# ToniChopp/ECAMP

Hardware: AMD Instinct MI355X
Metric: pretrain image-report pairs/sec (ViT-B/16, 224^2, seq=128) (higher is better)
Workload: dtype bf16

## Files before the change

ecamp_amd/csrc/core.hip:

```cpp
#include "common.h"
#include "attention.h"
#include "options.h"
#include "../../include/ecamp_hip.h"
#include <atomic>
#include <stdarg.h>
#include <stdlib.h>

thread_local char g_ecamp_err[512] = {0};

int ecamp_set_error(int code, const char* fmt, ...) {
    va_list ap;
    va_start(ap, fmt);
    vsnprintf(g_ecamp_err, sizeof(g_ecamp_err), fmt, ap);
    va_end(ap);
    return code;
}

extern "C" const char* ecamp_last_error(void) { return g_ecamp_err; }
extern "C" int ecamp_abi_version(void) { return ECAMP_ABI_VERSION; }
extern "C" int ecamp_half_format(void) { return ECAMP_HALF_IS_F16; }

#define OPT_UNREAD (INT_MIN + 1)
struct OptRow {
    const char* name; const char* env; int def; int (*set)(int);
    std::atomic<int> value{OPT_ENV};
    std::atomic<int> env_value{OPT_UNREAD};
};
static OptRow g_opts[OPT_COUNT] = {
              {"q8_mode", "ECAMP_GEMM_Q8", -1, [](int v) { return v == 0 || v == 2 ? v : -1; }},
               {"q8_sch", "ECAMP_Q8_SCH", 7, [](int v) { return v >= 0 ? v : OPT_ENV; }},
             {"q16_mode", "ECAMP_Q16", 1, [](int v) { return v >= 0 && v <= 3 ? v : OPT_ENV; }},
                {nullptr, "ECAMP_F8_Q8", 1, nullptr},
         {nullptr, "ECAMP_Q8_MIN_ITEMS", OPT_AUTO, nullptr},
          {"q8_bwd_grid", "ECAMP_Q8_BWD_GRID", 0, [](int v) { return v > 0 ? v : OPT_ENV; }},
             {"p8_wgrad", nullptr, 1, [](int v) { return v ? 1 : 0; }},
     {"p8_wgrad_reserve_cus", nullptr, 0, [](int v) { return v < 0 ? 0 : v; }},
          {nullptr, "ECAMP_WGRAD_ITEMS", 0, nullptr},
           {nullptr, "ECAMP_WGRAD_PLAN", 1, nullptr},
      {nullptr, "ECAMP_WGRAD_GROUP_CUS", 0, nullptr},
        {nullptr, "ECAMP_GEMM_GRID_CAP", 0, nullptr},
            {"attn_head", "ECAMP_ATTN_HEAD", 1, [](int v) { return v < 0 ? OPT_ENV : v ? 1 : 0; }},
           {nullptr, "ECAMP_ATTN_WAVES", 0, nullptr},
               {nullptr, "ECAMP_LN_BWD", 0, nullptr},
            {nullptr, "ECAMP_CE_KERNEL", 1, nullptr},
            {nullptr, "ECAMP_SR_BLOCKS", 512, nullptr},
};
int ecamp_opt_default(EcampOpt id) { return g_opts[id].def; }
int ecamp_opt(EcampOpt id) {
    OptRow& o = g_opts[id];
    const int s = o.value.load(std::memory_order_relaxed);
    if (s != OPT_ENV) return s;
    int e = o.env_value.load(std::memory_order_relaxed);
    if (e == OPT_UNREAD) {
        const char* txt = o.env ? getenv(o.env) : nullptr;
        e = txt ? atoi(txt) : o.def;
        o.env_value.store(e, std::memory_order_relaxed);
    }
    return e;
}
bool ecamp_opt_set(const char* name, int value) {
    for (OptRow& o : g_opts)
        if (o.name && strcmp(name, o.name) == 0) {
            o.value.store(o.set(value), std::memory_order_relaxed);
            return true;
        }
    return false;
}
extern "C" int ecamp_set_option(const char* name, int32_t value) {
    ECAMP_CHECK_ARG(name != nullptr, "set_option: null name");
    if (strcmp(name, "attn_head") == 0) { attn_set_head_mode(value); return 0; }
    if (ecamp_opt_set(name, value)) return 0;
    return ecamp_set_error(-1, "set_option: unknown option '%s'", name);
}

__global__ void dev_spin_kernel(long long cycles) {
    const long long t0 = clock64();
    while (clock64() - t0 < cycles) {}
}
extern "C" int ecamp_dev_spin(int32_t blocks, int32_t threads, int64_t cycles, hipStream_t stream) {
    ECAMP_CHECK_ARG(blocks > 0 && threads > 0 && threads <= 1024 && cycles >= 0, "dev_spin: bad arguments");
    hipLaunchKernelGGL(dev_spin_kernel, dim3(blocks), dim3(threads), 0, stream, (long long)cycles);
    ECAMP_LAUNCH_CHECK();
    return 0;
}
```

ecamp_amd/csrc/norm.hip:

```cpp
#include "common.h"
#include <initializer_list>

template <typename T, int VEC> struct LnVec;
template <> struct LnVec<float, 4> {
    typedef float4 raw_t;
    static __device__ __forceinline__ void cvt(const float4& v, float (&o)[4]) { o[0] = v.x; o[1] = v.y; o[2] = v.z; o[3] = v.w; }
    static __device__ __forceinline__ float4 pack(const float (&o)[4]) { return make_float4(o[0], o[1], o[2], o[3]); }
};
template <> struct LnVec<float, 8> {
    struct raw_t { float4 a, b; };
    static __device__ __forceinline__ void cvt(const raw_t& v, float (&o)[8]) {
        o[0] = v.a.x; o[1] = v.a.y; o[2] = v.a.z; o[3] = v.a.w; o[4] = v.b.x; o[5] = v.b.y; o[6] = v.b.z; o[7] = v.b.w;
    }
};
template <> struct LnVec<bf16_t, 4> {
    typedef uint2 raw_t;
    static __device__ __forceinline__ void cvt(const uint2& v, float (&o)[4]) {
        o[0] = h16_lo(v.x); o[1] = h16_hi(v.x);
        o[2] = h16_lo(v.y); o[3] = h16_hi(v.y);
    }
    static __device__ __forceinline__ uint2 pack(const float (&o)[4]) { return make_uint2(pack_bf16x2(o[0], o[1]), pack_bf16x2(o[2], o[3])); }
};
template <> struct LnVec<bf16_t, 8> {
    typedef uint4 raw_t;
    static __device__ __forceinline__ void cvt(const uint4& v, float (&o)[8]) {
        o[0] = h16_lo(v.x); o[1] = h16_hi(v.x);
        o[2] = h16_lo(v.y); o[3] = h16_hi(v.y);
        o[4] = h16_lo(v.z); o[5] = h16_hi(v.z);
        o[6] = h16_lo(v.w); o[7] = h16_hi(v.w);
    }
    static __device__ __forceinline__ uint4 pack(const float (&o)[8]) {
        return make_uint4(pack_bf16x2(o[0], o[1]), pack_bf16x2(o[2], o[3]), pack_bf16x2(o[4], o[5]), pack_bf16x2(o[6], o[7]));
    }
};
template <int VEC>
__device__ __forceinline__ void ln_dropout(uint64_t seed, uint64_t offset, long row, int nv, int c, float p, float inv_keep, float (&m)[VEC]) {
    if constexpr (VEC == 8) {
        dropout_scale8(seed, offset, (uint64_t)(row * nv + c), p, inv_keep, m);
    } else {
        static_assert(VEC == 4, "ln_dropout: 4- or 8-wide chunks");
        dropout_scale4(seed, offset, (uint64_t)(row * nv + c), p, inv_keep, m);
    }
}

template <typename T> struct ln_z32 {};
template <typename T> struct LnRow { typedef T io; typedef T z; };
template <typename T> struct LnRow<ln_z32<T>> { typedef T io; typedef float z; };

template <typename T, int IT, int VEC>
__global__ __launch_bounds__(256) void ln_fwd_kernel(const T* __restrict__ x, const T* __restrict__ res, T* __restrict__ zout,
                                                     const float* __restrict__ gamma, const float* __restrict__ beta,
                                                     T* __restrict__ y, float* __restrict__ mean, float* __restrict__ rstd,
                                                     long rows, int cols, float eps, float drop_p, uint64_t seed,
                                                     uint64_t offset, unsigned char* __restrict__ q8, const float* __restrict__ q8_scale,
                                                     float* __restrict__ q8_amax) {
    typedef typename LnRow<T>::io TY;
    typedef typename LnRow<T>::z TX;
    typedef LnVec<TY, VEC> V;
    typedef LnVec<TX, VEC> VX;
    typedef typename V::raw_t raw_t;
    const int lane = threadIdx.x & 63;
    const long row = (long)blockIdx.x * 4 + (threadIdx.x >> 6);
    if (row >= rows) return;
    const float q8_inv = q8 ? 1.0f / fmaxf(q8_scale[0], 1e-30f) : 0.f;
    float q8_max = 0.f;
    const int nv = cols / VEC;
    const float inv_keep = drop_p > 0.f ? 1.0f / (1.0f - drop_p) : 1.0f;
    typename VX::raw_t rx[IT];
    raw_t rr[IT];
#pragma unroll
    for (int i = 0; i < IT; ++i) {
        const int c = lane + 64 * i;
        if (c < nv) {
            rx[i] = *reinterpret_cast<const typename VX::raw_t*>(reinterpret_cast<const TX*>(x) + row * cols + c * VEC);
            if (res) rr[i] = *reinterpret_cast<const raw_t*>(reinterpret_cast<const TY*>(res) + row * cols + c * VEC);
        }
    }
    float v[IT][VEC];
    float s = 0.f;
#pragma unroll
    for (int i = 0; i < IT; ++i) {
        const int c = lane + 64 * i;
        if (c < nv) {
            VX::cvt(rx[i], v[i]);
            if (drop_p > 0.f) {
                float m[VEC];
                ln_dropout<VEC>(seed, offset, row, nv, c, drop_p, inv_keep, m);
#pragma unroll
                for (int r = 0; r < VEC; ++r) v[i][r] *= m[r];
            }
            if (res) {
                float q[VEC];
                V::cvt(rr[i], q);
#pragma unroll
                for (int r = 0; r < VEC; ++r) v[i][r] += q[r];
            }
            if (zout) {
#pragma unroll
                for (int r = 0; r < VEC; ++r) v[i][r] = rnd<TY>(v[i][r]);
                *reinterpret_cast<raw_t*>(reinterpret_cast<TY*>(zout) + row * cols + c * VEC) = V::pack(v[i]);
            }
#pragma unroll
            for (int r = 0; r < VEC; r += 4) s += (v[i][r] + v[i][r + 1]) + (v[i][r + 2] + v[i][r + 3]);
        } else {
#pragma unroll
            for (int r = 0; r < VEC; ++r) v[i][r] = 0.f;
        }
    }
    const float mu = wave_sum(s) / (float)cols;
    float q = 0.f;
#pragma unroll
    for (int i = 0; i < IT; ++i) {
        const int c = lane + 64 * i;
        if (c < nv) {
#pragma unroll
            for (int r = 0; r < VEC; ++r) {
                const float d = v[i][r] - mu;
                q += d * d;
            }
        }
    }
    const float rs = rsqrtf(wave_sum(q) / (float)cols + eps);
    if (lane == 0) {
        mean[row] = mu;
        rstd[row] = rs;
    }
#pragma unroll
    for (int i = 0; i < IT; ++i) {
        const int c = lane + 64 * i;
        if (c < nv) {
            float o[VEC];
#pragma unroll
            for (int k = 0; k < VEC / 4; ++k) {
                const float4 g = *reinterpret_cast<const float4*>(gamma + c * VEC + 4 * k);
                const float4 b = *reinterpret_cast<const float4*>(beta + c * VEC + 4 * k);
                o[4 * k + 0] = (v[i][4 * k + 0] - mu) * rs * g.x + b.x;
                o[4 * k + 1] = (v[i][4 * k + 1] - mu) * rs * g.y + b.y;
                o[4 * k + 2] = (v[i][4 * k + 2] - mu) * rs * g.z + b.z;
                o[4 * k + 3] = (v[i][4 * k + 3] - mu) * rs * g.w + b.w;
            }
            *reinterpret_cast<raw_t*>(reinterpret_cast<TY*>(y) + row * cols + c * VEC) = V::pack(o);
            if (q8) {
                unsigned int w[VEC / 4];
#pragma unroll
                for (int k = 0; k < VEC / 4; ++k) {
                    float u[4];
#pragma unroll
                    for (int r = 0; r < 4; ++r) {
                        const float yr = rnd<TY>(o[4 * k + r]);
                        q8_max = fmaxf(q8_max, fabsf(yr));
                        u[r] = fminf(fmaxf(yr * q8_inv, -448.f), 448.f);
                    }
                    int ww = 0;
                    ww = __builtin_amdgcn_cvt_pk_fp8_f32(u[0], u[1], ww, false);
                    ww = __builtin_amdgcn_cvt_pk_fp8_f32(u[2], u[3], ww, true);
                    w[k] = (unsigned int)ww;
                }
                if constexpr (VEC == 8) *reinterpret_cast<uint2*>(q8 + row * cols + c * VEC) = make_uint2(w[0], w[1]);
                else *reinterpret_cast<unsigned int*>(q8 + row * cols + c * VEC) = w[0];
            }
        }
    }
    if (q8) {
        q8_max = wave_max(q8_max);
        if (lane == 0) atomicMax(reinterpret_cast<unsigned int*>(q8_amax + (blockIdx.x & 15) * 32), __float_as_uint(q8_max));
    }
}

template <typename T, int IT, int VEC, int LN_BWD_WAVES, bool GREG>
__global__ __launch_bounds__(LN_BWD_WAVES * 64) void ln_bwd_kernel(const T* __restrict__ dy, const T* __restrict__ z,
                                                     const float* __restrict__ mean, const float* __restrict__ rstd,
                                                     const float* __restrict__ gamma, const T* __restrict__ dres,
                                                     T* __restrict__ dz, T* __restrict__ dxdrop, float* __restrict__ dgamma,
                                                     float* __restrict__ dbeta, long rows, int cols, float drop_p,
                                                     uint64_t seed, uint64_t offset) {
    typedef typename LnRow<T>::io TY;
    typedef typename LnRow<T>::z TZ;
    typedef LnVec<TY, VEC> V;
    typedef LnVec<TZ, VEC> VZ;
    typedef typename V::raw_t raw_t;
    typedef typename VZ::raw_t zraw_t;
    extern __shared__ __attribute__((aligned(16))) float sh[];
    const int lane = threadIdx.x & 63, wave = threadIdx.x >> 6;
    const int nv = cols / VEC;
    const float inv_keep = drop_p > 0.f ? 1.0f / (1.0f - drop_p) : 1.0f;
    float ag[IT][VEC], ab[IT][VEC];
    float gmr[GREG ? IT : 1][VEC];
    float* shg = sh + 8 * cols;
#pragma unroll
    for (int i = 0; i < IT; ++i) {
        const int c = lane + 64 * i;
#pragma unroll
        for (int r = 0; r < VEC; ++r) ag[i][r] = ab[i][r] = 0.f;
        if (GREG) {
#pragma unroll
            for (int k = 0; k < VEC / 4; ++k) {
                const float4 g4 = c < nv ? *reinterpret_cast<const float4*>(gamma + c * VEC + 4 * k) : make_float4(0.f, 0.f, 0.f, 0.f);
                gmr[i][4 * k] = g4.x; gmr[i][4 * k + 1] = g4.y; gmr[i][4 * k + 2] = g4.z; gmr[i][4 * k + 3] = g4.w;
            }
        }
    }
    if (!GREG) {
        for (int c = threadIdx.x; c < cols; c += LN_BWD_WAVES * 64) shg[c] = gamma[c];
        __syncthreads();
    }
    auto gam = [&](int i, int c, int k, float (&o4)[4]) __attribute__((always_inline)) {
        if (GREG) { o4[0] = gmr[GREG ? i : 0][4 * k]; o4[1] = gmr[GREG ? i : 0][4 * k + 1]; o4[2] = gmr[GREG ? i : 0][4 * k + 2]; o4[3] = gmr[GREG ? i : 0][4 * k + 3]; }
        else { const float4 g4 = *reinterpret_cast<const float4*>(shg + c * VEC + 4 * k); o4[0] = g4.x; o4[1] = g4.y; o4[2] = g4.z; o4[3] = g4.w; }
    };
    raw_t rdy[IT];
    zraw_t rz[IT];
    raw_t rq[IT];
    float nmu = 0.f, nrs = 0.f;
    const long stride = (long)gridDim.x * LN_BWD_WAVES;
    auto fetch = [&](long row) {
        nmu = mean[row];
        nrs = rstd[row];
#pragma unroll
        for (int i = 0; i < IT; ++i) {
            const int c = lane + 64 * i;
            if (c < nv) {
                rdy[i] = *reinterpret_cast<const raw_t*>(reinterpret_cast<const TY*>(dy) + ((unsigned)(row * cols) + (unsigned)(c * VEC)));
                rz[i] = *reinterpret_cast<const zraw_t*>(reinterpret_cast<const TZ*>(z) + ((unsigned)(row * cols) + (unsigned)(c * VEC)));
            }
        }
    };
    auto fetch_q = [&](long row) {
#pragma unroll
        for (int i = 0; i < IT; ++i) {
            const int c = lane + 64 * i;
            if (c < nv) rq[i] = *reinterpret_cast<const raw_t*>(reinterpret_cast<const TY*>(dres) + ((unsigned)(row * cols) + (unsigned)(c * VEC)));
        }
    };
    long row = (long)blockIdx.x * LN_BWD_WAVES + wave;
    if (row < rows) { fetch(row); if (dres) fetch_q(row); }
    for (; row < rows; row += stride) {
        const float mu = nmu, rs = nrs;
        raw_t cdy[IT];
        zraw_t cz[IT];
        float s1 = 0.f, s2 = 0.f;
#pragma unroll
        for (int i = 0; i < IT; ++i) {
            const int c = lane + 64 * i;
            cdy[i] = rdy[i]; cz[i] = rz[i];
            if (c < nv) {
                float d[VEC], zz[VEC], gm[VEC];
                V::cvt(cdy[i], d);
                VZ::cvt(cz[i], zz);
#pragma unroll
                for (int k = 0; k < VEC / 4; ++k) {
                    float g4[4];
                    gam(i, c, k, g4);
                    gm[4 * k] = g4[0]; gm[4 * k + 1] = g4[1]; gm[4 * k + 2] = g4[2]; gm[4 * k + 3] = g4[3];
                }
#pragma unroll
                for (int r = 0; r < VEC; ++r) {
                    const float xh = (zz[r] - mu) * rs, g = d[r] * gm[r];
                    s1 += g;
                    s2 += g * xh;
                    ag[i][r] += d[r] * xh;
                    ab[i][r] += d[r];
                }
            }
        }
        if (row + stride < rows) fetch(row + stride);
        s1 = wave_sum(s1) / (float)cols;
        s2 = wave_sum(s2) / (float)cols;
#pragma unroll
        for (int i = 0; i < IT; ++i) {
            const int c = lane + 64 * i;
            if (c < nv) {
                float d[VEC], zz[VEC], o[VEC];
                V::cvt(cdy[i], d);
                VZ::cvt(cz[i], zz);
#pragma unroll
                for (int k = 0; k < VEC / 4; ++k) {
                    float gm[4];
                    gam(i, c, k, gm);
#pragma unroll
                    for (int r = 0; r < 4; ++r) {
                        const float xh = (zz[4 * k + r] - mu) * rs, g = d[4 * k + r] * gm[r];
                        o[4 * k + r] = rs * (g - s1 - xh * s2);
                    }
                }
                if (dres) {
                    float q[VEC];
                    V::cvt(rq[i], q);
#pragma unroll
                    for (int r = 0; r < VEC; ++r) o[r] += q[r];
                }
                *reinterpret_cast<raw_t*>(reinterpret_cast<TY*>(dz) + ((unsigned)(row * cols) + (unsigned)(c * VEC))) = V::pack(o);
                if (dxdrop) {
                    if (drop_p > 0.f) {
                        float m[VEC];
                        ln_dropout<VEC>(seed, offset, row, nv, c, drop_p, inv_keep, m);
#pragma unroll
                        for (int r = 0; r < VEC; ++r) o[r] = rnd<TY>(o[r]) * m[r];
                    }
                    *reinterpret_cast<raw_t*>(reinterpret_cast<TY*>(dxdrop) + ((unsigned)(row * cols) + (unsigned)(c * VEC))) = V::pack(o);
                }
            }
        }
        if (dres && row + stride < rows) fetch_q(row + stride);
    }
    for (int pass = 0; pass < 2; ++pass) {
        float tot[2] = {0.f, 0.f};
        for (int half = 0; half < (LN_BWD_WAVES + 7) / 8; ++half) {
            const int nsl = LN_BWD_WAVES - 8 * half < 8 ? LN_BWD_WAVES - 8 * half : 8;
            __syncthreads();
            if ((wave >> 3) == half) {
#pragma unroll
                for (int i = 0; i < IT; ++i) {
                    const int c = lane + 64 * i;
                    if (c < nv) {
#pragma unroll
                        for (int k = 0; k < VEC / 4; ++k)
                            *reinterpret_cast<float4*>(sh + (wave & 7) * cols + c * VEC + 4 * k) =
                                pass == 0 ? make_float4(ag[i][4 * k], ag[i][4 * k + 1], ag[i][4 * k + 2], ag[i][4 * k + 3])
                                          : make_float4(ab[i][4 * k], ab[i][4 * k + 1], ab[i][4 * k + 2], ab[i][4 * k + 3]);
                    }
                }
            }
            __syncthreads();
#pragma unroll
            for (int j = 0; j < 2; ++j) {
                const int c = threadIdx.x + j * LN_BWD_WAVES * 64;
                if (c < cols) {
#pragma unroll
                    for (int w = 0; w < 8; ++w) if (w < nsl) tot[j] += sh[w * cols + c];
                }
            }
        }
        float* dst = pass == 0 ? dgamma : dbeta;
#pragma unroll
        for (int j = 0; j < 2; ++j) {
            const int c = threadIdx.x + j * LN_BWD_WAVES * 64;
            if (c < cols) atomicAdd(dst + c, tot[j]);
        }
    }
}

struct LnLayout {
    int vec;
    int chunks;
    int waves;
    bool greg;
    size_t lds;
    int grid_cap;
};

static bool ln_al16(std::initializer_list<const void*> ptrs) {
    for (const void* q : ptrs)
        if (reinterpret_cast<uintptr_t>(q) & 15) return false;
    return true;
}

static LnLayout ln_select(bool backward, bool rows16, int cols, bool al16, int opt_bwd) {
    const bool wide = rows16 && cols % 8 == 0 && al16;
    const int it8 = ceil_div(cols / 8, 64), it4 = ceil_div(cols / 4, 64);
    const int chunks4 = it4 <= 1 ? 1 : it4 <= 4 ? it4 : 8;
    if (!backward) return {wide ? 8 : 4, !wide ? chunks4 : it8 <= 1 ? 1 : it8 <= 2 ? 2 : 4, 4, true, 0, 0};
    const size_t slices = (size_t)8 * cols * sizeof(float);
    if (wide && opt_bwd != 1 && cols <= 1024) {
        if (it8 <= 1) return {8, 1, 16, true, slices, 256};
        if (opt_bwd == 2 || cols > 768) return {8, 2, 12, false, (size_t)9 * cols * sizeof(float), 256};
    }
    return {4, chunks4, 16, true, slices, 256};
}

template <typename T> constexpr bool ln_rows16 = sizeof(typename LnRow<T>::io) == 2;

template <typename T>
static void ln_fwd_launch(const void* x, const void* res, void* z, const float* gamma, const float* beta, void* y, float* mean,
                          float* rstd, long rows, int cols, float eps, float p, uint64_t seed, uint64_t off, hipStream_t st,
                          void* q8 = nullptr, const float* q8_scale = nullptr, float* q8_amax = nullptr) {
    const LnLayout l = ln_select(false, ln_rows16<T>, cols, ln_al16({x, res, z, y}), 0);
    auto k = ln_fwd_kernel<T, 8, 4>;
    if (l.vec == 4) {
        k = l.chunks == 1 ? ln_fwd_kernel<T, 1, 4> : l.chunks == 2 ? ln_fwd_kernel<T, 2, 4> : l.chunks == 3 ? ln_fwd_kernel<T, 3, 4>
          : l.chunks == 4 ? ln_fwd_kernel<T, 4, 4> : k;
    } else if constexpr (ln_rows16<T>) {
        k = l.chunks == 1 ? ln_fwd_kernel<T, 1, 8> : l.chunks == 2 ? ln_fwd_kernel<T, 2, 8> : ln_fwd_kernel<T, 4, 8>;
    }
    hipLaunchKernelGGL(k, dim3(ceil_div(rows, l.waves)), dim3(l.waves * 64), l.lds, st, (const T*)x, (const T*)res, (T*)z, gamma, beta, (T*)y,
                       mean, rstd, rows, cols, eps, p, seed, off, (unsigned char*)q8, q8_scale, q8_amax);
}

template <typename T>
static void ln_bwd_launch(const void* dy, const void* z, const float* mean, const float* rstd, const float* gamma, const void* dres,
                          void* dz, void* dxdrop, float* dgamma, float* dbeta, long rows, int cols, float p, uint64_t seed,
                          uint64_t off, int opt_bwd, hipStream_t st) {
    const LnLayout l = ln_select(true, ln_rows16<T>, cols, ln_al16({dy, z, dres, dz, dxdrop}), opt_bwd);
    auto k = ln_bwd_kernel<T, 8, 4, 16, true>;
    if (l.vec == 4) {
        k = l.chunks == 1 ? ln_bwd_kernel<T, 1, 4, 16, true> : l.chunks == 2 ? ln_bwd_kernel<T, 2, 4, 16, true>
          : l.chunks == 3 ? ln_bwd_kernel<T, 3, 4, 16, true> : l.chunks == 4 ? ln_bwd_kernel<T, 4, 4, 16, true> : k;
    } else if constexpr (ln_rows16<T>) {
        k = l.chunks == 1 ? ln_bwd_kernel<T, 1, 8, 16, true> : ln_bwd_kernel<T, 2, 8, 12, false>;
    }
    int nb = ceil_div(rows, l.waves);
    if (nb > l.grid_cap) nb = l.grid_cap;
    hipLaunchKernelGGL(k, dim3(nb), dim3(l.waves * 64), l.lds, st, (const T*)dy, (const T*)z, mean, rstd, gamma, (const T*)dres, (T*)dz,
                       (T*)dxdrop, dgamma, dbeta, rows, cols, p, seed, off);
}

extern "C" int ecamp_layernorm_fwd(const void* x, const void* residual, void* z_out, const float* gamma, const float* beta,
                                   void* y, float* mean, float* rstd, int64_t rows, int32_t cols, float eps, float drop_p,
                                   uint64_t seed, uint64_t offset, int32_t dtype, hipStream_t stream) {
    ECAMP_CHECK_ARG(x && gamma && beta && y && mean && rstd, "layernorm_fwd: null pointer");
    ECAMP_CHECK_ARG(cols % 4 == 0 && cols <= 2048 && rows > 0, "layernorm_fwd: cols=%d must be a multiple of 4 and <= 2048", cols);
    ECAMP_CHECK_ARG(!(residual || drop_p > 0.f) || z_out, "layernorm_fwd: fused residual/dropout needs z_out");
    if (dtype == ECAMP_F32) ln_fwd_launch<float>(x, residual, z_out, gamma, beta, y, mean, rstd, rows, cols, eps, drop_p, seed, offset, stream);
    else if (dtype == ECAMP_BF16) ln_fwd_launch<bf16_t>(x, residual, z_out, gamma, beta, y, mean, rstd, rows, cols, eps, drop_p, seed, offset, stream);
    else return ecamp_set_error(-1, "layernorm_fwd: bad dtype %d", dtype);
    ECAMP_LAUNCH_CHECK();
    return 0;
}

extern "C" int ecamp_layernorm_fwd_q8(const void* x, const void* residual, void* z_out, const float* gamma, const float* beta,
                                      void* y, float* mean, float* rstd, int64_t rows, int32_t cols, float eps, float drop_p,
                                      uint64_t seed, uint64_t offset, void* q8, const float* q8_scale, float* q8_amax_slots,
                                      int32_t dtype, hipStream_t stream) {
    ECAMP_CHECK_ARG(x && gamma && beta && y && mean && rstd && q8 && q8_scale && q8_amax_slots, "layernorm_fwd_q8: null pointer");
    ECAMP_CHECK_ARG(cols % 4 == 0 && cols <= 2048 && rows > 0, "layernorm_fwd_q8: cols=%d must be a multiple of 4 and <= 2048", cols);
    ECAMP_CHECK_ARG(!(residual || drop_p > 0.f) || z_out, "layernorm_fwd_q8: fused residual/dropout needs z_out");
    ECAMP_CHECK_ARG(dtype == ECAMP_BF16 && (reinterpret_cast<uintptr_t>(q8) & 7) == 0, "layernorm_fwd_q8: bf16 rows, 8-byte aligned q8");
    ln_fwd_launch<bf16_t>(x, residual, z_out, gamma, beta, y, mean, rstd, rows, cols, eps, drop_p, seed, offset, stream, q8, q8_scale, q8_amax_slots);
    ECAMP_LAUNCH_CHECK();
    return 0;
}

extern "C" int ecamp_layernorm_bwd(const void* dy, const void* z, const float* mean, const float* rstd, const float* gamma,
                                   const void* dres_in, void* dz, void* dx_drop, float* dgamma, float* dbeta, int64_t rows,
                                   int32_t cols, float drop_p, uint64_t seed, uint64_t offset, int32_t dtype,
                                   hipStream_t stream) {
    ECAMP_CHECK_ARG(dy && z && mean && rstd && gamma && dz && dgamma && dbeta, "layernorm_bwd: null pointer");
    ECAMP_CHECK_ARG(cols % 4 == 0 && cols <= 2048 && rows > 0, "layernorm_bwd: cols=%d must be a multiple of 4 and <= 2048", cols);
    ECAMP_CHECK_ARG(rows * (int64_t)cols < (1ll << 30), "layernorm_bwd: rows * cols must stay below 2^30 (32-bit element offsets)");
    const int opt = ecamp_opt(OPT_LN_BWD);
    if (dtype == ECAMP_F32) ln_bwd_launch<float>(dy, z, mean, rstd, gamma, dres_in, dz, dx_drop, dgamma, dbeta, rows, cols, drop_p, seed, offset, opt, stream);
    else if (dtype == ECAMP_BF16) ln_bwd_launch<bf16_t>(dy, z, mean, rstd, gamma, dres_in, dz, dx_drop, dgamma, dbeta, rows, cols, drop_p, seed, offset, opt, stream);
    else return ecamp_set_error(-1, "layernorm_bwd: bad dtype %d", dtype);
    ECAMP_LAUNCH_CHECK();
    return 0;
}

extern "C" int ecamp_layernorm_fwd_x32(const float* x, const float* gamma, const float* beta, void* y, float* mean, float* rstd, int64_t rows,
                                       int32_t cols, float eps, int32_t dtype, hipStream_t stream) {
    ECAMP_CHECK_ARG(x && gamma && beta && y && mean && rstd, "layernorm_fwd_x32: null pointer");
    ECAMP_CHECK_ARG(cols % 4 == 0 && cols <= 2048 && rows > 0, "layernorm_fwd_x32: cols=%d must be a multiple of 4 and <= 2048", cols);
    ECAMP_CHECK_ARG(dtype == ECAMP_BF16, "layernorm_fwd_x32: the output is 16-bit (dtype 1), got %d", dtype);
    ECAMP_CHECK_ARG((reinterpret_cast<uintptr_t>(x) & 15) == 0 && (reinterpret_cast<uintptr_t>(y) & 7) == 0, "layernorm_fwd_x32: x 16-B, y 8-B aligned");
    ln_fwd_launch<ln_z32<bf16_t>>(x, nullptr, nullptr, gamma, beta, y, mean, rstd, rows, cols, eps, 0.f, 0, 0, stream);
    ECAMP_LAUNCH_CHECK();
    return 0;
}

extern "C" int ecamp_layernorm_bwd_z32(const void* dy, const float* z, const float* mean, const float* rstd, const float* gamma, const void* dres_in,
                                       void* dz, float* dgamma, float* dbeta, int64_t rows, int32_t cols, int32_t dtype, hipStream_t stream) {
    ECAMP_CHECK_ARG(dy && z && mean && rstd && gamma && dz && dgamma && dbeta, "layernorm_bwd_z32: null pointer");
    ECAMP_CHECK_ARG(cols % 4 == 0 && cols <= 2048 && rows > 0, "layernorm_bwd_z32: cols=%d must be a multiple of 4 and <= 2048", cols);
    ECAMP_CHECK_ARG(rows * (int64_t)cols < (1ll << 30), "layernorm_bwd_z32: rows * cols must stay below 2^30 (32-bit element offsets)");
    ECAMP_CHECK_ARG(dtype == ECAMP_BF16, "layernorm_bwd_z32: dy / dres / dz are 16-bit (dtype 1), got %d", dtype);
    ECAMP_CHECK_ARG((reinterpret_cast<uintptr_t>(z) & 15) == 0, "layernorm_bwd_z32: z 16-B aligned");
    ln_bwd_launch<ln_z32<bf16_t>>(dy, z, mean, rstd, gamma, dres_in, dz, nullptr, dgamma, dbeta, rows, cols, 0.f, 0, 0, 0, stream);
    ECAMP_LAUNCH_CHECK();
    return 0;
}
```

ecamp_amd/csrc/options.h:

```cpp
#pragma once
#include <limits.h>

enum EcampOpt {
    OPT_Q8_MODE, OPT_Q8_SCH, OPT_Q16_MODE, OPT_F8_Q8, OPT_Q8_MIN_ITEMS, OPT_Q8_BWD_GRID, OPT_P8_WGRAD, OPT_P8_WGRAD_RESERVE,
    OPT_WGRAD_ITEMS, OPT_WGRAD_PLAN, OPT_WGRAD_GROUP_CUS, OPT_GEMM_GRID_CAP, OPT_ATTN_HEAD, OPT_ATTN_WAVES, OPT_LN_BWD, OPT_CE_KERNEL,
    OPT_SR_BLOCKS, OPT_COUNT
};
#define OPT_ENV INT_MIN
#define OPT_AUTO INT_MIN

#define ECAMP_HIDDEN __attribute__((visibility("hidden")))
ECAMP_HIDDEN int ecamp_opt(EcampOpt id);
ECAMP_HIDDEN int ecamp_opt_default(EcampOpt id);
ECAMP_HIDDEN bool ecamp_opt_set(const char* name, int value);
```

Baseline: 7355.

## Use atomic work-claiming for dynamic row scheduling in LayerNorm backward

Replaces the static grid-stride row loop in the LayerNorm backward kernel with dynamic work stealing. Each workgroup claims chunks of rows through a global atomic ticket, and each wave processes several contiguous rows per claim. The aim is to balance load across CUs when the grid is capped and rows do not divide evenly, and to improve locality with contiguous rows per wave. In exchange it adds global atomics and an extra __syncthreads per claimed block, plus a slot-reset protocol that relies on a ring of 1024 device counter slots.

Measured after the change: 7381, median of 4. About the same (+0.4%).

```diff
diff --git a/ecamp_amd/csrc/core.hip b/ecamp_amd/csrc/core.hip
--- a/ecamp_amd/csrc/core.hip
+++ b/ecamp_amd/csrc/core.hip
@@ -42,6 +42,7 @@
             {"attn_head", "ECAMP_ATTN_HEAD", 1, [](int v) { return v < 0 ? OPT_ENV : v ? 1 : 0; }},
            {nullptr, "ECAMP_ATTN_WAVES", 0, nullptr},
                {nullptr, "ECAMP_LN_BWD", 0, nullptr},
+         {"ln_bwd_claim", "ECAMP_LN_BWD_CLAIM", 1, [](int v) { return v < 0 ? OPT_ENV : v ? 1 : 0; }},
             {nullptr, "ECAMP_CE_KERNEL", 1, nullptr},
             {nullptr, "ECAMP_SR_BLOCKS", 512, nullptr},
 };
diff --git a/ecamp_amd/csrc/norm.hip b/ecamp_amd/csrc/norm.hip
--- a/ecamp_amd/csrc/norm.hip
+++ b/ecamp_amd/csrc/norm.hip
@@ -1,4 +1,6 @@
 #include "common.h"
+#include <algorithm>
+#include <atomic>
 #include <initializer_list>
 
 template <typename T, int VEC> struct LnVec;
@@ -167,13 +169,24 @@
     }
 }
 
+constexpr int LN_CLAIM_SLOTS = 1024;
+constexpr int LN_CLAIMS_PER_WG = 4;
+__device__ unsigned int g_ln_claim[LN_CLAIM_SLOTS][2];
+
+__device__ __forceinline__ void ln_claim_exit(unsigned int* slot) {
+    if (__hip_atomic_fetch_add(slot + 1, 1u, __ATOMIC_RELAXED, __HIP_MEMORY_SCOPE_AGENT) == gridDim.x - 1) {
+        __hip_atomic_store(slot, 0u, __ATOMIC_RELAXED, __HIP_MEMORY_SCOPE_AGENT);
+        __hip_atomic_store(slot + 1, 0u, __ATOMIC_RELAXED, __HIP_MEMORY_SCOPE_AGENT);
+    }
+}
+
 template <typename T, int IT, int VEC, int LN_BWD_WAVES, bool GREG>
 __global__ __launch_bounds__(LN_BWD_WAVES * 64) void ln_bwd_kernel(const T* __restrict__ dy, const T* __restrict__ z,
                                                      const float* __restrict__ mean, const float* __restrict__ rstd,
                                                      const float* __restrict__ gamma, const T* __restrict__ dres,
                                                      T* __restrict__ dz, T* __restrict__ dxdrop, float* __restrict__ dgamma,
                                                      float* __restrict__ dbeta, long rows, int cols, float drop_p,
-                                                     uint64_t seed, uint64_t offset) {
+                                                     uint64_t seed, uint64_t offset, int slot, int rpb) {
     typedef typename LnRow<T>::io TY;
     typedef typename LnRow<T>::z TZ;
     typedef LnVec<TY, VEC> V;
@@ -182,6 +195,21 @@
     typedef typename VZ::raw_t zraw_t;
     extern __shared__ __attribute__((aligned(16))) float sh[];
     const int lane = threadIdx.x & 63, wave = threadIdx.x >> 6;
+    const bool claim = slot >= 0;
+    unsigned int* const ticket = &g_ln_claim[claim ? slot : 0][0];
+    unsigned int* const tk = reinterpret_cast<unsigned int*>(sh);
+    const unsigned int bstep = (unsigned int)(LN_BWD_WAVES * rpb);
+    long cur = (long)blockIdx.x * LN_BWD_WAVES, nxt = cur + (long)gridDim.x * LN_BWD_WAVES;
+    if (claim) {
+        if (threadIdx.x == 0) tk[1] = __hip_atomic_fetch_add(ticket, 2 * bstep, __ATOMIC_RELAXED, __HIP_MEMORY_SCOPE_AGENT);
+        __syncthreads();
+        cur = (long)(unsigned int)__builtin_amdgcn_readfirstlane(tk[1]);
+        if (cur >= rows) {
+            if (threadIdx.x == 0) ln_claim_exit(ticket);
+            return;
+        }
+        nxt = cur + bstep;
+    }
     const int nv = cols / VEC;
     const float inv_keep = drop_p > 0.f ? 1.0f / (1.0f - drop_p) : 1.0f;
     float ag[IT][VEC], ab[IT][VEC];
@@ -212,7 +240,6 @@
     zraw_t rz[IT];
     raw_t rq[IT];
     float nmu = 0.f, nrs = 0.f;
-    const long stride = (long)gridDim.x * LN_BWD_WAVES;
     auto fetch = [&](long row) {
         nmu = mean[row];
         nrs = rstd[row];
@@ -232,9 +259,23 @@
             if (c < nv) rq[i] = *reinterpret_cast<const raw_t*>(reinterpret_cast<const TY*>(dres) + ((unsigned)(row * cols) + (unsigned)(c * VEC)));
         }
     };
-    long row = (long)blockIdx.x * LN_BWD_WAVES + wave;
-    if (row < rows) { fetch(row); if (dres) fetch_q(row); }
-    for (; row < rows; row += stride) {
+    const long wrow = (long)(wave * rpb);
+    if (cur + wrow < rows) { fetch(cur + wrow); if (dres) fetch_q(cur + wrow); }
+    unsigned int drawn = 0;
+    for (unsigned int blk = 0; cur < rows; ++blk) {
+      if (claim && threadIdx.x == 0) {
+        drawn = (unsigned int)nxt;
+        if (nxt < rows) {
+            unsigned long long t = reinterpret_cast<unsigned long long>(ticket);
+            asm volatile("" : "+v"(t));
+            drawn = __hip_atomic_fetch_add(reinterpret_cast<__attribute__((address_space(1))) unsigned int*>(t), bstep, __ATOMIC_RELAXED,
+                                           __HIP_MEMORY_SCOPE_AGENT);
+        }
+      }
+      for (int j = 0; j < rpb; ++j) {
+        const long row = cur + wrow + j;
+        if (row >= rows) break;
+        const long nrow = j + 1 < rpb ? row + 1 : nxt + wrow;
         const float mu = nmu, rs = nrs;
         raw_t cdy[IT];
         zraw_t cz[IT];
@@ -263,7 +304,7 @@
                 }
             }
         }
-        if (row + stride < rows) fetch(row + stride);
+        if (nrow < rows) fetch(nrow);
         s1 = wave_sum(s1) / (float)cols;
         s2 = wave_sum(s2) / (float)cols;
 #pragma unroll
@@ -301,7 +342,16 @@
                 }
             }
         }
-        if (dres && row + stride < rows) fetch_q(row + stride);
+        if (dres && nrow < rows) fetch_q(nrow);
+      }
+      cur = nxt;
+      if (claim) {
+        if (threadIdx.x == 0) tk[blk & 1] = drawn;
+        __syncthreads();
+        nxt = (long)(unsigned int)__builtin_amdgcn_readfirstlane(tk[blk & 1]);
+      } else {
+        nxt += (long)gridDim.x * LN_BWD_WAVES;
+      }
     }
     for (int pass = 0; pass < 2; ++pass) {
         float tot[2] = {0.f, 0.f};
@@ -338,6 +388,7 @@
             if (c < cols) atomicAdd(dst + c, tot[j]);
         }
     }
+    if (claim && threadIdx.x == 0) ln_claim_exit(ticket);
 }
 
 struct LnLayout {
@@ -398,10 +449,17 @@
     } else if constexpr (ln_rows16<T>) {
         k = l.chunks == 1 ? ln_bwd_kernel<T, 1, 8, 16, true> : ln_bwd_kernel<T, 2, 8, 12, false>;
     }
-    int nb = ceil_div(rows, l.waves);
+    static std::atomic<unsigned int> next_slot{0};
+    int slot = -1, rpb = 1;
+    if (ecamp_opt(OPT_LN_BWD_CLAIM)) {
+        const long quad = (long)LN_CLAIMS_PER_WG * l.waves * l.grid_cap;
+        rpb = (int)std::max(1l, (rows + quad / 2) / quad);
+        slot = (int)(next_slot.fetch_add(1, std::memory_order_relaxed) % LN_CLAIM_SLOTS);
+    }
+    int nb = ceil_div(rows, (long)l.waves * rpb);
     if (nb > l.grid_cap) nb = l.grid_cap;
     hipLaunchKernelGGL(k, dim3(nb), dim3(l.waves * 64), l.lds, st, (const T*)dy, (const T*)z, mean, rstd, gamma, (const T*)dres, (T*)dz,
-                       (T*)dxdrop, dgamma, dbeta, rows, cols, p, seed, off);
+                       (T*)dxdrop, dgamma, dbeta, rows, cols, p, seed, off, slot, rpb);
 }
 
 extern "C" int ecamp_layernorm_fwd(const void* x, const void* residual, void* z_out, const float* gamma, const float* beta,
diff --git a/ecamp_amd/csrc/options.h b/ecamp_amd/csrc/options.h
--- a/ecamp_amd/csrc/options.h
+++ b/ecamp_amd/csrc/options.h
@@ -3,8 +3,8 @@
 
 enum EcampOpt {
     OPT_Q8_MODE, OPT_Q8_SCH, OPT_Q16_MODE, OPT_F8_Q8, OPT_Q8_MIN_ITEMS, OPT_Q8_BWD_GRID, OPT_P8_WGRAD, OPT_P8_WGRAD_RESERVE,
-    OPT_WGRAD_ITEMS, OPT_WGRAD_PLAN, OPT_WGRAD_GROUP_CUS, OPT_GEMM_GRID_CAP, OPT_ATTN_HEAD, OPT_ATTN_WAVES, OPT_LN_BWD, OPT_CE_KERNEL,
-    OPT_SR_BLOCKS, OPT_COUNT
+    OPT_WGRAD_ITEMS, OPT_WGRAD_PLAN, OPT_WGRAD_GROUP_CUS, OPT_GEMM_GRID_CAP, OPT_ATTN_HEAD, OPT_ATTN_WAVES, OPT_LN_BWD, OPT_LN_BWD_CLAIM,
+    OPT_CE_KERNEL, OPT_SR_BLOCKS, OPT_COUNT
 };
 #define OPT_ENV INT_MIN
 #define OPT_AUTO INT_MIN
```
